# tangle-network/zk-SaaS

Measured on AMD Instinct MI355X. Metric: Groth16 proofs/sec (SHA-256 circuit), higher is better.
Workload: dtype u32 limbs (256-bit Montgomery); 1 GPU; BASELINE configs[3]: full distributed Groth16 on the SHA-256 circuit, BN254, l=2, n=8 parties on one GPU, all 12 masks sampled and applied (sha256.rs:226-291); masks=True, constraints=30006, wires=29823, domain=32768, len_a=14911, len_w=14911, len_u=16384, parties=8, packing_factor=2, fixed_base_tables=True

## Files before the change

### zk-saas_amd/csrc/msm.hpp

```cpp
#pragma once
#include <algorithm>
#include <atomic>
#include <cstdio>
#include <cstdlib>
#include <future>
#include <map>
#include <memory>
#include <mutex>
#include <type_traits>
#include <vector>

#include "ec.hpp"
#include "engine.hpp"
#include "msm_plan.hpp"
#include "ntt.hpp"
#include "quad.hpp"

namespace zk {
#if defined(__HIPCC__)

enum MsmRole { ROLE_SH, ROLE_W, ROLE_V, ROLE_U, NROLES };
constexpr const char* ROLE_NAME[NROLES] = {"S+H", "W", "V", "U"};
constexpr int NJOBS = 2;
constexpr int NBATCH = 3;
// ... 970 lines not shown
        k++;
        end_k = end_n;
        while (end_k == p + 1) {
          k++;
          end_k = offsets[k + 1];
        }
        end_n = offsets[k + 2 <= nkeys ? k + 2 : nkeys];
      }
    }
    e = e_next;
    pt = pt_next;
  }
}

constexpr int QUAD_THREADS = 256;
constexpr int QUAD_VL = QUAD_THREADS / 4;
inline int quad_threads(bool batched) {
  return batched ? 64 : 256;
}

template <class Fld>
__global__ __launch_bounds__(64) void msm_heavy_kernel(const XYZZ<Fld>* __restrict__ edge0, uint32_t nlanes, uint32_t tmin,
                                                       uint32_t cap, const uint32_t* __restrict__ offsets, uint32_t nkeys,
                                                       XYZZ<Fld>* __restrict__ buckets0,
                                                       const uint32_t* __restrict__ heavy,
                                                       XYZZ<Fld>* __restrict__ hpart0, uint32_t vcap, size_t ys) {
  __builtin_amdgcn_s_setprio(3);
  ZK_YSHIFT(offsets);
  ZK_YSHIFT(heavy);
  const uint32_t nh = heavy[1], V = heavy[0];
  if (blockIdx.x >= V) return;
  const XYZZ<Fld>* __restrict__ head = edge0 + (size_t)blockIdx.y * 2 * nlanes;
  const XYZZ<Fld>* __restrict__ tail = head + nlanes;
  XYZZ<Fld>* __restrict__ buckets = buckets0 + (size_t)blockIdx.y * nkeys;
  XYZZ<Fld>* __restrict__ hpart = hpart0 + (size_t)blockIdx.y * vcap;
  extern __shared__ uint4 smem_fin[];
  XYZZ<Fld>* sh = reinterpret_cast<XYZZ<Fld>*>(smem_fin);
  const uint32_t T = msm_range_len(offsets[nkeys], nlanes, tmin, cap);
  const int q = threadIdx.x & 3, vl = threadIdx.x >> 2;
  const int nq = (int)blockDim.x / 4;
  for (uint32_t v = blockIdx.x; v < V; v += gridDim.x) {
    uint32_t lo = 0, hi = nh;
    while (hi - lo > 1) {
      const uint32_t mid = (lo + hi) >> 1;
      if (heavy[3 + 2 * mid] <= v) lo = mid;
      else hi = mid;
    }
    const uint32_t kh = heavy[2 + 2 * lo], vb = heavy[3 + 2 * lo];
    const uint32_t S = (lo + 1 < nh ? heavy[3 + 2 * (lo + 1)] : V) - vb, s = v - vb;
    const uint32_t o0 = offsets[kh], o1 = offsets[kh + 1];
    const uint32_t l0 = o0 / T, l1 = (o1 - 1) / T;
    const uint32_t chunk = (l1 - l0 + S - 1) / S;
    const uint32_t first = l0 + 1 + s * chunk, last = first + chunk - 1 < l1 ? first + chunk - 1 : l1;
    Fld acc = (s == 0 && vl == 0) ? qload(tail + l0, q) : qidentity<Fld>(q);
    for (uint32_t l = first + (uint32_t)vl; l <= last; l += (uint32_t)nq) acc = qadd(acc, qload(head + l, q), q);
    acc = wg_quad_sum(acc, sh, vl, q, nq);
    if (vl == 0) qstore(S == 1 ? buckets + kh : hpart + v, q, acc);
    __syncthreads();
  }
}

constexpr int FIN_THREADS = 64;
template <class Fld>
__global__ __launch_bounds__(FIN_THREADS) void msm_finalize_kernel(const XYZZ<Fld>* __restrict__ edge0, uint32_t nlanes,
                                                               uint32_t tmin, uint32_t cap,
                                                               const uint32_t* __restrict__ offsets, uint32_t nkeys,
                                                               XYZZ<Fld>* __restrict__ buckets0,
                                                               const uint32_t* __restrict__ heavy,
                                                               const XYZZ<Fld>* __restrict__ hpart0, uint32_t vcap,
                                                               uint32_t fin_wgs, size_t ys) {
  __builtin_amdgcn_s_setprio(3);
  ZK_YSHIFT(offsets);
  const XYZZ<Fld>* __restrict__ head = edge0 + (size_t)blockIdx.y * 2 * nlanes;
  const XYZZ<Fld>* __restrict__ tail = head + nlanes;
  XYZZ<Fld>* __restrict__ buckets = buckets0 + (size_t)blockIdx.y * nkeys;
  const int q = threadIdx.x & 3;
  if (blockIdx.x >= fin_wgs) {
    ZK_YSHIFT(heavy);
    const uint32_t nh = heavy[1], V = heavy[0];
    const XYZZ<Fld>* __restrict__ hpart = hpart0 + (size_t)blockIdx.y * vcap;
    extern __shared__ uint4 smem_fin[];
    XYZZ<Fld>* sh = reinterpret_cast<XYZZ<Fld>*>(smem_fin);
    const int vl = threadIdx.x >> 2;
    for (uint32_t h = blockIdx.x - fin_wgs; h < nh; h += gridDim.x - fin_wgs) {
      const uint32_t vb = heavy[3 + 2 * h], S = (h + 1 < nh ? heavy[3 + 2 * (h + 1)] : V) - vb;
      if (S == 1) continue;
      Fld acc = qidentity<Fld>(q);
      for (uint32_t j = (uint32_t)vl; j < S; j += FIN_THREADS / 4) acc = qadd(acc, qload(hpart + vb + j, q), q);
      acc = wg_quad_sum(acc, sh, vl, q, FIN_THREADS / 4);
      if (vl == 0) qstore(buckets + heavy[2 + 2 * h], q, acc);
      __syncthreads();
    }
    return;
  }
  const uint32_t T = msm_range_len(offsets[nkeys], nlanes, tmin, cap);
  for (size_t k = (size_t)blockIdx.x * (FIN_THREADS / 4) + (threadIdx.x >> 2); k < nkeys;
       k += (size_t)fin_wgs * (FIN_THREADS / 4)) {
    const uint32_t o0 = offsets[k], o1 = offsets[k + 1];
    if (o0 == o1) {
      qstore(buckets + k, q, qidentity<Fld>(q));
      continue;
    }
    const uint32_t l0 = o0 / T, l1 = (o1 - 1) / T;
    if (l1 == l0 || l1 - l0 > FIN_SEQ) continue;
    Fld acc = qload(tail + l0, q);
    for (uint32_t l = l0 + 1; l <= l1; l++) acc = qadd(acc, qload(head + l, q), q);
    qstore(buckets + k, q, acc);
  }
}

template <class Fld>
__global__ __launch_bounds__(QUAD_THREADS, 2) void msm_reduce_a_kernel(const XYZZ<Fld>* __restrict__ buckets0, uint32_t B,
                                                                   int lo_bits, int nvl, XYZZ<Fld>* __restrict__ out0) {
  __builtin_amdgcn_s_setprio(3);
  extern __shared__ uint4 smem_red[];
  XYZZ<Fld>* sh = reinterpret_cast<XYZZ<Fld>*>(smem_red);
  const uint32_t LO = 1u << lo_bits, HI = B >> lo_bits;
  const uint32_t ngroups = HI + 1 + LO;
  const XYZZ<Fld>* __restrict__ wb = buckets0 + (size_t)blockIdx.y * B;
  const int q = threadIdx.x & 3, vl = threadIdx.x >> 2;
  const uint32_t g = blockIdx.x * (uint32_t)((int)blockDim.x / 4 / nvl) + (uint32_t)(vl / nvl);
  const uint32_t sub = (uint32_t)(vl & (nvl - 1));
  Fld acc = qidentity<Fld>(q);
  if (g <= HI) {
    for (uint32_t lo = sub; lo < LO; lo += (uint32_t)nvl) {
      uint32_t k = g * LO + lo;
      if (k >= 1 && k <= B) acc = qadd(acc, qload(wb + (k - 1), q), q);
    }
  } else if (g < ngroups) {
    const uint32_t lo = g - HI - 1;
    for (uint32_t hi = sub; hi <= HI; hi += (uint32_t)nvl) {
      uint32_t k = hi * LO + lo;
      if (k >= 1 && k <= B) acc = qadd(acc, qload(wb + (k - 1), q), q);
    }
  }
  acc = wg_quad_sum(acc, sh, vl, q, nvl);
  if (sub == 0 && g < ngroups) qstore(out0 + (size_t)blockIdx.y * ngroups + g, q, acc);
}

template <class Fld>
__global__ __launch_bounds__(QUAD_THREADS, 2) void msm_reduce_b_kernel(const XYZZ<Fld>* __restrict__ rc0, uint32_t B, int lo_bits,
                                                                   int nvl, XYZZ<Fld>* __restrict__ out0,
                                                                   const uint32_t* __restrict__ cnt_src, size_t cnt_stride,
                                                                   uint32_t ncnt, uint32_t* __restrict__ cnt_dst) {
  __builtin_amdgcn_s_setprio(3);
  if (blockIdx.x == 0 && blockIdx.y == 0 && threadIdx.x < ncnt)
    cnt_dst[2 * threadIdx.x] = *(const uint32_t*)((const char*)cnt_src + threadIdx.x * cnt_stride);
  extern __shared__ uint4 smem_red[];
  XYZZ<Fld>* sh = reinterpret_cast<XYZZ<Fld>*>(smem_red);
  const uint32_t LO = 1u << lo_bits, HI = B >> lo_bits;
  const uint32_t ngroups = HI + 1 + LO;
  int hb = 0;
  while ((1u << hb) < HI) hb++;
  const int nslices = hb + 1 + lo_bits;
  const XYZZ<Fld>* __restrict__ rc = rc0 + (size_t)blockIdx.y * ngroups;
  const int q = threadIdx.x & 3, vl = threadIdx.x >> 2;
  const int j = (int)blockIdx.x * ((int)blockDim.x / 4 / nvl) + vl / nvl;
  const uint32_t sub = (uint32_t)(vl & (nvl - 1));
  Fld acc = qidentity<Fld>(q);
  if (j <= hb) {
    for (uint32_t hi = sub; hi <= HI; hi += (uint32_t)nvl)
      if ((hi >> j) & 1u) acc = qadd(acc, qload(rc + hi, q), q);
  } else if (j < nslices) {
    const int jj = j - hb - 1;
    for (uint32_t lo = sub; lo < LO; lo += (uint32_t)nvl)
      if ((lo >> jj) & 1u) acc = qadd(acc, qload(rc + HI + 1 + lo, q), q);
  }
  acc = wg_quad_sum(acc, sh, vl, q, nvl);
  if (sub == 0 && j < nslices) qstore(out0 + (size_t)blockIdx.y * nslices + j, q, acc);
}

template <class Fld>
__global__ __launch_bounds__(128) void msm_table_kernel(const Affine<Fld>* __restrict__ bases, size_t len, int c,
                                                       int nwin, int wide, Affine<Fld>* __restrict__ table) {
  size_t i = (size_t)blockIdx.x * blockDim.x + threadIdx.x;
  if (i >= len) return;
  Affine<Fld> p = load_elem(bases + i);
  if (p.is_identity()) {
    for (int w = 0; w < nwin; w++) store_elem(table + (size_t)w * len + i, p);
    return;
  }
  XYZZ<Fld> acc = XYZZ<Fld>::from_affine(p);
  int left = 0;
  for (int w = 0; w < nwin;) {
    if (left == 0) {
      store_elem(table + (size_t)w * len + i, xyzz_to_affine(acc));
      left = w < wide ? c : c - 1;
      w++;
      if (w == nwin) break;
    }
    acc = xyzz_dbl(acc);
    left--;
  }
}

#endif

template <class Fld>
struct KernelField {
  using type = Fld;
};
template <class P>
struct KernelField<Fp2T<P, false>> {
  using type = Fp2T<P, (P::N <= ZK_MUL_INLINE_LIMBS)>;
};

struct MsmSlot {
  DevBuf ws;
  void* pinned = nullptr;
  size_t pinned_bytes = 0;
  hipEvent_t ev = nullptr;
  std::atomic<bool> busy{false};
  std::shared_ptr<const MsmTable> tab, tab2;
  hipError_t wait(const IEngine* eng) {
    if (!busy) return hipSuccess;
    hipError_t he = eng->event_wait(ev);
    if (he == hipErrorNotReady) return he;
    tab.reset();
    tab2.reset();
    busy = false;
    return he;
  }
// ... 426 lines not shown
```

### zk-saas_amd/csrc/msm_impl.hpp

```cpp
#pragma once
#include "msm.hpp"
#include "pack_split.hpp"

namespace zk {

#define MSM_HIP(x)                                           \
  do {                                                       \
    hipError_t _e = (x);                                     \
    if (_e != hipSuccess) return eng->hip_fail(_e, #x);      \
  } while (0)
#ifdef ZK_MSM_DEBUG_SYNC
#define MSM_STAGE(name)                                                          \
  do {                                                                           \
    hipError_t _e = hipStreamSynchronize(st);                                    \
    fprintf(stderr, "[zk msm] %s done (%s) npts=%zu c=%d nwin=%d\n", name,       \
            hipGetErrorString(_e), pl.npts, pl.win.c, pl.win.nwin);              \
    if (_e != hipSuccess) return eng->hip_fail(_e, name);                        \
  } while (0)
#else
#define MSM_STAGE(name) do { } while (0)
#endif

template <class Fr, class KF>
struct MsmViews {
// ... 104 lines not shown
                                           std::to_string(gate.sorted_cnt->load()) + " of " + std::to_string(gate.sorted_need) + ")");
    for (int i = 0; i < gate.n_wait_sorted; i++) MSM_HIP(hipStreamWaitEvent(st, gate.wait_sorted[i], 0));
  }
  if (gate.wait_ev) {
    if (gate.wait_flag && !eng->spin_until([&] { return gate.wait_flag->load(std::memory_order_acquire) != 0; }))
      return eng->fail(ZK_ERR_GENERIC, "msm launch: the accumulate kernel ahead of this one in the batch's chain was not enqueued within the deadline");
    MSM_HIP(hipStreamWaitEvent(st, gate.wait_ev, 0));
  }
  if constexpr (G2FLD) {
    msm_accumulate_split_kernel<typename BaseParams<Fld>::type><<<dim3((nlanes + 31) / 32, NB), dim3(128), 0, st>>>(
        bases, bases2, v.sorted, v.offsets, nkeys, nlanes, pl.tmin, pl.cap, v.buckets, v.edge, v.heavy, v.k0, pl.ys);
  } else {
    msm_accumulate_kernel<KF><<<dim3((nlanes + 127) / 128, NB), dim3(128), 0, st>>>(
        (const Affine<KF>*)bases, (const Affine<KF>*)bases2, v.sorted, v.offsets, nkeys, nlanes, pl.tmin, pl.cap, v.buckets,
        v.edge, v.heavy, v.k0, pl.ys, 0);
  }
  if (gate.signal_ev) {
    MSM_HIP(hipEventRecord(gate.signal_ev, st));
    if (gate.signal_flag) gate.signal_flag->store(1, std::memory_order_release);
  }
  return ZK_OK;
}

template <class Fr, class Fld, class KF>
int msm_stage_reduce(IEngine* eng, const MsmPlan& pl, const MsmViews<Fr, KF>& v, hipStream_t st) {
  constexpr bool G2FLD = IsExtField<Fld>::value;
  const unsigned NB = pl.vectors, nsets = (unsigned)pl.nsets;
  const uint32_t nkeys = (uint32_t)pl.nkeys, nlanes = pl.nlanes, tmin = pl.tmin, cap = pl.cap;
  const size_t ys = pl.ys;
  ProfScope ps_(eng->prof, G2FLD ? PROF_MSM_REDUCE_G2 : PROF_MSM_REDUCE, st, (double)pl.nkeys * NB);
  const int qt = quad_threads(pl.batch > 1), qvl = qt / 4;
  const size_t quad_lds = (size_t)qvl * sizeof(XYZZ<Fld>);
  msm_heavy_kernel<KF><<<dim3(2048, NB), dim3(64), (size_t)16 * sizeof(XYZZ<Fld>), st>>>(v.edge, nlanes, tmin, cap, v.offsets, nkeys,
                                                                    v.buckets, v.heavy, v.hpart, pl.vcap, ys);
  MSM_STAGE("heavy buckets");
  {
    const size_t fin_wgs = std::min<size_t>((pl.nkeys + FIN_THREADS / 4 - 1) / (FIN_THREADS / 4), 8192);
    const unsigned fin_extra = 256;
    msm_finalize_kernel<KF><<<dim3((unsigned)fin_wgs + fin_extra, NB), dim3(FIN_THREADS),
                              (size_t)(FIN_THREADS / 4) * sizeof(XYZZ<Fld>), st>>>(
        v.edge, nlanes, tmin, cap, v.offsets, nkeys, v.buckets, v.heavy, v.hpart, pl.vcap, (uint32_t)fin_wgs, ys);
  }
  MSM_STAGE("finalize");
  const size_t tot_groups = (size_t)pl.red_groups * NB * nsets;
  const size_t tot_slices = (size_t)pl.nslices * NB * nsets;
  const size_t cap_quads = (size_t)1024 * (G2FLD ? 2 : 3) * 16;
  auto pick_nvl = [&](size_t groups) {
    int n = qvl;
    while (n > 4 && groups * (size_t)n > cap_quads) n >>= 1;
    return n;
  };
  const int nvl_a = pick_nvl(tot_groups), nvl_b = pick_nvl(tot_slices);
  const unsigned gpw_a = (unsigned)(qvl / nvl_a), gpw_b = (unsigned)(qvl / nvl_b);
  msm_reduce_a_kernel<KF><<<dim3((pl.red_groups + gpw_a - 1) / gpw_a, NB * nsets), dim3((unsigned)qt), quad_lds, st>>>(
      v.buckets, pl.B, pl.lo_bits, nvl_a, v.rc);
  msm_reduce_b_kernel<KF><<<dim3(((unsigned)pl.nslices + gpw_b - 1) / gpw_b, NB * nsets), dim3((unsigned)qt), quad_lds, st>>>(
      v.rc, pl.B, pl.lo_bits, nvl_b, v.out,
      v.offsets + nkeys, ys, pl.nsorts, v.stats);
  return ZK_OK;
}

template <class FrP, class Fld>
int msm_launch(IEngine* eng, MsmSlot& slot, const MsmTuning& tune, const void* bases, const void* bases2,
               const void* scalars, size_t npts, const Fp<FrP>* coef_d, size_t part_len, hipStream_t st,
               MsmPending* pend, const MsmBatchArg* ba) {
  using Fr = Fp<FrP>;
  using KF = typename KernelField<Fld>::type;
  static_assert(sizeof(KF) == sizeof(Fld), "kernel field layout");
  static_assert(sizeof(XYZZ<Fld>) == 4 * sizeof(Fld), "the plan sizes XYZZ points as four coordinates");
  constexpr bool G2FLD = IsExtField<Fld>::value;
  *pend = MsmPending{};
  const unsigned NB = bases2 ? 2u : 1u;
  const void* const bases_in = bases;
  const void* const bases2_in = bases2;
  size_t toff = 0, toff2 = 0;
  std::shared_ptr<const MsmTable> tab = TableRegistry::inst().find(bases, npts, sizeof(Affine<Fld>), FrP::BITS, &toff), tab2;
  if (tab && NB == 2) {
    tab2 = TableRegistry::inst().find(bases2, npts, sizeof(Affine<Fld>), FrP::BITS, &toff2);
    if (!tab2 || tab2->len != tab->len || toff2 != toff || tab2->c != tab->c) tab = nullptr;
    else bases2 = tab2->data;
  }
  if (tab) bases = tab->data;
  MsmPlanIn in;
  in.scalar_bits = FrP::BITS, in.scalar_bytes = (int)sizeof(Fr), in.coord_bytes = (int)sizeof(Fld), in.g2 = G2FLD;
  if constexpr (G2FLD) in.acc_waves = SPLIT_WAVES<typename BaseParams<Fld>::type>;
  else in.acc_waves = ACC_WAVES<Fld>;
  in.npts = npts, in.batch = ba ? (size_t)ba->nb : 1, in.vectors = (int)NB;
  if (tab) {
    in.tab_c = tab->c, in.tab_len = tab->len, in.tab_off = toff;
    in.tab_no_identity = !tab->any_identity && (NB == 1 || !tab2->any_identity);
  }
  in.c_force = tune.c_force, in.bigsort_min = tune.bigsort_min;
  const MsmPlan pl = msm_plan(in);
  if (pl.err) return eng->fail(ZK_ERR_BAD_INPUT, pl.err);
  pend->fold = pl.fold;
  if (npts == 0) return ZK_OK;
  hipError_t he = slot.ws.ensure(pl.ws_bytes);
  if (he != hipSuccess) return eng->hip_fail(he, "msm workspace");
  he = slot.ensure_pinned(pl.pinned_bytes);
  if (he != hipSuccess) return eng->hip_fail(he, "msm pinned buffer");
  if (!slot.ev) {
    he = hipEventCreateWithFlags(&slot.ev, hipEventDisableTiming);
    if (he != hipSuccess) return eng->hip_fail(he, "msm event");
  }
  slot.busy = true;
  slot.tab = tab;
  slot.tab2 = tab2;
  pend->slot = &slot;
  struct RecordOnExit {
    MsmSlot& s;
// ... 92 lines not shown
```

### zk-saas_amd/csrc/quad.hpp

```cpp
#pragma once
#include "ec.hpp"
#include "ntt.hpp"

namespace zk {
#if defined(__HIPCC__)

template <int P0, int P1, int P2, int P3>
ZK_D uint32_t qperm_u32(uint32_t v) {
  return (uint32_t)__builtin_amdgcn_mov_dpp((int)v, P0 | (P1 << 2) | (P2 << 4) | (P3 << 6), 0xf, 0xf, true);
}
template <int P0, int P1, int P2, int P3, class P>
ZK_D Fp<P> qperm(const Fp<P>& v) {
  Fp<P> r;
#pragma unroll
  for (int i = 0; i < P::N; i++) r.v[i] = qperm_u32<P0, P1, P2, P3>(v.v[i]);
  return r;
}
template <int P0, int P1, int P2, int P3, class P, bool I>
ZK_D Fp2T<P, I> qperm(const Fp2T<P, I>& v) {
  return {qperm<P0, P1, P2, P3>(v.c0), qperm<P0, P1, P2, P3>(v.c1)};
}
template <class P>
ZK_D Fp<P> qsel(bool a, const Fp<P>& x, const Fp<P>& y) {
  Fp<P> r;
#pragma unroll
  for (int i = 0; i < P::N; i++) r.v[i] = a ? x.v[i] : y.v[i];
  return r;
}
template <class P, bool I>
ZK_D Fp2T<P, I> qsel(bool a, const Fp2T<P, I>& x, const Fp2T<P, I>& y) {
  return {qsel(a, x.c0, y.c0), qsel(a, x.c1, y.c1)};
}

template <class Fld>
ZK_D Fld qidentity(int q) {
  return q < 2 ? Fld::one() : Fld::zero();
}
template <class Fld>
ZK_D Fld qload(const XYZZ<Fld>* p, int q) {
  return load_elem(reinterpret_cast<const Fld*>(p) + q);
}
template <class Fld>
ZK_D void qstore(XYZZ<Fld>* p, int q, const Fld& c) {
  store_elem(reinterpret_cast<Fld*>(p) + q, c);
}

template <class Fld>
ZK_D Fld qadd(const Fld& ca, const Fld& cb, int q) {
  const bool even = (q & 1) == 0;
  const bool za = qperm<2, 2, 2, 2>(ca).is_zero();
  const bool zb = qperm<2, 2, 2, 2>(cb).is_zero();
  Fld A = qsel(even, qperm<0, 0, 1, 1>(ca), qperm<0, 0, 1, 1>(cb));
  Fld B = qsel(even, qperm<2, 2, 3, 3>(cb), qperm<2, 2, 3, 3>(ca));
  const Fld m1 = A * B;
  const Fld d = qperm<1, 1, 3, 3>(m1) - qperm<0, 0, 2, 2>(m1);
  const bool pz = qperm<0, 0, 0, 0>(d).is_zero();
  const bool rz = qperm<2, 2, 2, 2>(d).is_zero();
  const bool D = pz && rz && !za && !zb;
  const Fld cu = qsel(q == 1, ca.dbl(), ca);
  A = qsel(D, cu, qsel(even, d, qperm<0, 2, 2, 3>(ca)));
  B = qsel(D, cu, qsel(even, d, qperm<0, 2, 2, 3>(cb)));
  const Fld m2 = A * B;
  const Fld XX = qperm<0, 0, 0, 0>(m2);
  const Fld M = XX.dbl() + XX;
  A = qsel(D, qsel(q == 3, M, cu), qsel(q == 2, qperm<0, 1, 1, 3>(m2), qsel(q == 1, d, m1)));
  B = qsel(D, qsel(q == 3, M, qperm<1, 1, 1, 1>(m2)), XX);
  const Fld m3 = A * B;
  const Fld m3_1 = qperm<1, 1, 1, 1>(m3);
  const Fld m3_0 = qperm<0, 0, 0, 0>(m3);
  const Fld T = qsel(D, qperm<3, 3, 3, 3>(m3), qperm<2, 2, 2, 2>(m2)) - m3_0.dbl();
  const Fld X3f = qsel(D, T, T - m3_1);
  A = qsel(D, qsel(q == 0, M, m3_1),
           qsel(q == 1, qperm<2, 2, 2, 2>(d), qsel(q == 0, qperm<2, 2, 2, 2>(m1), m2)));
  B = qsel(D, qsel(q == 0, m3_0 - X3f, ca),
           qsel(q == 1, m3_0 - X3f, m3_1));
  const Fld m4 = A * B;
  const Fld m4_0 = qperm<0, 0, 0, 0>(m4), m4_1 = qperm<1, 1, 1, 1>(m4);
  const Fld Y3 = qsel(D, m4_0 - m4_1, m4_1 - m4_0);
  Fld r = qsel(q == 0, X3f, qsel(q == 1, Y3, qsel(q == 2, m3, m4)));
  if (pz && !rz) r = qidentity<Fld>(q);
  if (zb) r = ca;
  if (za) r = cb;
  return r;
}

template <class F>
ZK_D F cswap(const F& v) {
  return qperm<1, 0, 3, 2>(v);
}
template <class F>
ZK_D F hswap(const F& v) {
  return qperm<2, 3, 0, 1>(v);
}
template <class P>
ZK_D Fp<P> s2_mul(const Fp<P>& a, const Fp<P>& b, bool comp) {
  const Fp<P> ao = cswap(a), bo = cswap(b);
  return Fp<P>::mul_pm_mul(a, qsel(comp, bo, b), ao, qsel(comp, b, bo), comp);
}
template <class P>
ZK_D Fp<P> s2_sqr(const Fp<P>& a, bool comp) {
  const Fp<P> ao = cswap(a);
  return (a + qsel(comp, a, ao)) * qsel(comp, ao, a - ao);
}
template <class P>
ZK_D bool s2_is_zero(const Fp<P>& a) {
  const uint32_t z = a.is_zero() ? 1u : 0u;
  return (z & qperm_u32<1, 0, 3, 2>(z)) != 0;
}
template <class P>
struct SplitAcc {
  Fp<P> c0, c1;
};
template <class P>
ZK_D SplitAcc<P> split_identity(bool comp) {
  return SplitAcc<P>{qsel(comp, Fp<P>::zero(), Fp<P>::one()), Fp<P>::zero()};
}
template <class P>
ZK_D SplitAcc<P> split_madd(const SplitAcc<P>& a, const Fp<P>& in, bool half, bool comp) {
  using F = Fp<P>;
  const uint32_t zz = s2_is_zero(a.c1) ? 1u : 0u;
  SplitAcc<P> r;
  if (qperm_u32<0, 0, 0, 0>(zz)) {
    r.c0 = in;
    r.c1 = qsel(comp, F::zero(), F::one());
    return r;
  }
  const F m1 = s2_mul(in, a.c1, comp);
  const F d = m1 - a.c0;
  const F od = hswap(d);
  const uint32_t dz = s2_is_zero(d) ? 1u : 0u;
  const bool pz = qperm_u32<0, 0, 0, 0>(dz) != 0, rz = qperm_u32<2, 2, 2, 2>(dz) != 0;
  if (pz) {
    if (!rz) return split_identity<P>(comp);
    const F u = qsel(half, in.dbl(), in);
    const F m2 = s2_sqr(u, comp);
    const F o2 = hswap(m2);
// ... 46 lines not shown
  const Fp<P> ninv = (sq + cswap(sq)).inverse_fast();
  const Fp<P> r = z * ninv;
  return qsel(comp, r.neg(), r);
}
ZK_D bool quad_all(bool b) {
  uint32_t z = b ? 1u : 0u;
  z &= qperm_u32<1, 0, 3, 2>(z);
  z &= qperm_u32<2, 3, 0, 1>(z);
  return z != 0;
}
template <class P>
__device__ __noinline__ Fp<P> split_affine_add(const Fp<P>& a, bool ida, const Fp<P>& b, bool idb, bool half, bool comp,
                                               bool* idr) {
  using F = Fp<P>;
  *idr = false;
  if (ida) {
    *idr = idb;
    return b;
  }
  if (idb) return a;
  const F d = b - a;
  const uint32_t dz = s2_is_zero(d) ? 1u : 0u;
  const bool xz = qperm_u32<0, 0, 0, 0>(dz) != 0, yz = qperm_u32<2, 2, 2, 2>(dz) != 0;
  const F xa = qperm<0, 1, 0, 1>(a), ya = qperm<2, 3, 2, 3>(a);
  F lam;
  if (xz) {
    if (!yz) {
      *idr = true;
      return F::zero();
    }
    const F xx = s2_sqr(xa, comp);
    lam = s2_mul(xx.dbl() + xx, split_inv(ya.dbl(), comp), comp);
  } else {
    lam = s2_mul(qperm<2, 3, 2, 3>(d), split_inv(qperm<0, 1, 0, 1>(d), comp), comp);
  }
  const F x3 = s2_sqr(lam, comp) - xa - qperm<0, 1, 0, 1>(b);
  const F y3 = s2_mul(lam, xa - x3, comp) - ya;
  return qsel(half, y3, x3);
}

template <class P>
ZK_D void split_store_affine(const SplitAcc<P>& acc, Fp<P>* dst, bool half, bool comp) {
  using F = Fp<P>;
  const uint32_t zz = s2_is_zero(acc.c1) ? 1u : 0u;
  if (qperm_u32<0, 0, 0, 0>(zz)) {
    store_elem(dst, F::zero());
    return;
  }
  const F zi = split_inv(qperm<2, 3, 2, 3>(acc.c1), comp);
  const F zi2 = s2_sqr(s2_mul(zi, qperm<0, 1, 0, 1>(acc.c1), comp), comp);
  store_elem(dst, s2_mul(acc.c0, qsel(half, zi, zi2), comp));
}

template <class Fld>
ZK_D Fld wg_quad_sum(Fld c, XYZZ<Fld>* sh, int vl, int q, int nvl) {
  qstore(sh + vl, q, c);
  __syncthreads();
  for (int off = nvl >> 1; off >= 1; off >>= 1) {
    const bool act = (vl & (nvl - 1)) < off;
    Fld r = c;
    if (act) r = qadd(c, qload(sh + vl + off, q), q);
    __syncthreads();
    if (act) {
      c = r;
      qstore(sh + vl, q, c);
    }
    __syncthreads();
  }
  return c;
}

#endif
}
```

### zk-saas_amd/csrc/msm_plan.hpp

```cpp
#pragma once
#include <algorithm>
#include <cstddef>
#include <cstdint>

namespace zk {

constexpr size_t MSM_RANGE_MIN = 20, MSM_RANGE = 64;
constexpr size_t MSM_RANGE_MIN_G2 = 16, MSM_RANGE_G2 = 64;
constexpr uint32_t FIN_SEQ = 16;
constexpr int MSM_MAXB = 16;

constexpr int BIG_HI = 8;
constexpr int BIG_MAX_BINS = 8192;
constexpr int BIG_THREADS = 256;
constexpr int BIG_PTS_PER_THREAD = 8;
constexpr int BIG_EPT = 16;
constexpr size_t BIG_LDS_MAX = 156 * 1024;
inline int msm_big_hi(size_t nsets) {
  int hi = BIG_HI;
  while (hi > 0 && (nsets << hi) > (size_t)BIG_MAX_BINS) hi--;
  return hi;
}
constexpr size_t msm_bins_words(size_t nbins) { return 3 * nbins + 2; }

constexpr int ISCAN_THREADS = 256;
constexpr int ISCAN_PER = 8;
constexpr int ISCAN_BLOCK = ISCAN_THREADS * ISCAN_PER;

inline size_t msm_heavy_cap(size_t nlanes) { return nlanes / FIN_SEQ + 8; }
inline size_t msm_heavy_vcap(size_t nlanes) { return nlanes / FIN_SEQ + nlanes / 256 + 8; }

struct MsmWindows {
  int c = 0, nwin = 0, wide = 0;
  static MsmWindows of(int scalar_bits, int c_req) {
    const int T = scalar_bits + 1;
    MsmWindows w;
    w.nwin = (T + c_req - 1) / c_req;
    w.c = (T + w.nwin - 1) / w.nwin;
    w.wide = T - w.nwin * (w.c - 1);
    return w;
  }
  int width(int w) const { return w < wide ? c : c - 1; }
  int start(int w) const { return w * (c - 1) + std::min(w, wide); }
};

inline int msm_pick_c(int scalar_bits, size_t npts, int c_force = 0) {
  if (c_force >= 2 && c_force <= 20) return c_force;
  int best = 4;
  double best_cost = 1e300;
  for (int c = 4; c <= 20; c++) {
    int nwin = (scalar_bits + c) / c;
    int ceff = (scalar_bits + nwin) / nwin;
    double cost = (double)nwin * ((double)npts + (ceff > 17 ? 10.0 : 4.0) * (double)((size_t)1 << (ceff - 1)));
    if (cost <= best_cost) {
      best_cost = cost;
      best = c;
    }
  }
  return best;
}

struct MsmLanes {
  uint32_t nlanes, tmin, cap;
};
inline MsmLanes msm_pick_lanes(size_t max_entries, int waves, bool pair, int lanes_per_range = 0) {
  if (!lanes_per_range) lanes_per_range = pair ? 2 : 1;
  const size_t cap = (size_t)1024 * waves * (64 / lanes_per_range);
  const size_t lo = pair ? MSM_RANGE_MIN_G2 : MSM_RANGE_MIN;
  const size_t hi = pair ? MSM_RANGE_G2 : MSM_RANGE;
  size_t t = std::min(hi, std::max(lo, (size_t)((double)max_entries / (2.4 * (double)cap))));
  size_t nl = std::max<size_t>(1, (max_entries + t - 1) / t);
  if (max_entries >= cap * t && max_entries < 2 * cap * t && (max_entries + 2 * cap - 1) / (2 * cap) >= 12)
    nl = std::max(nl, 2 * cap);
  return MsmLanes{(uint32_t)nl, (uint32_t)t, (uint32_t)cap};
}

inline int table_c_auto(size_t len, bool g2) {
  if (g2) return len < ((size_t)1 << 20) ? 15 : 19;
  return len <= ((size_t)1 << 17) ? 15 : len < ((size_t)1 << 19) ? 16 : len < ((size_t)1 << 22) ? 18 : 20;
}
// ... 222 lines not shown
```

Before: 647.9 proofs/s.

## Unify MSM chain and tree reductions into a single qadd call site

Replaces the separate accumulate-loop plus wg_quad_sum tree reduction with quad_chain_tree_sum, a single loop in which each step performs one qadd, first over chained addends and then over the LDS tree. The two bucket-reduce kernels are merged into one stage-parameterized msm_reduce_kernel, and the finalize kernel's heavy and normal paths now share that loop. The likely aim is to inline the large qadd body once per kernel to cut code size and register pressure. A per-type FIN_WAVES occupancy hint is added to the finalize kernel's launch bounds. In exchange there is more predicated, divergent work per step and extra barriers in the finalize path.

```diff
diff --git a/zk-saas_amd/csrc/msm.hpp b/zk-saas_amd/csrc/msm.hpp
--- a/zk-saas_amd/csrc/msm.hpp
+++ b/zk-saas_amd/csrc/msm.hpp
@@ -1047,8 +1047,12 @@
     const uint32_t chunk = (l1 - l0 + S - 1) / S;
     const uint32_t first = l0 + 1 + s * chunk, last = first + chunk - 1 < l1 ? first + chunk - 1 : l1;
     Fld acc = (s == 0 && vl == 0) ? qload(tail + l0, q) : qidentity<Fld>(q);
-    for (uint32_t l = first + (uint32_t)vl; l <= last; l += (uint32_t)nq) acc = qadd(acc, qload(head + l, q), q);
-    acc = wg_quad_sum(acc, sh, vl, q, nq);
+    const uint32_t nchain = last >= first ? (last - first + (uint32_t)nq) / (uint32_t)nq : 0;
+    acc = quad_chain_tree_sum(acc, nchain, nq, sh, vl, q, [&](uint32_t i, bool* valid) {
+      const uint32_t l = first + (uint32_t)vl + i * (uint32_t)nq;
+      *valid = l <= last;
+      return head + l;
+    });
     if (vl == 0) qstore(S == 1 ? buckets + kh : hpart + v, q, acc);
     __syncthreads();
   }
@@ -1056,7 +1060,9 @@
 
 constexpr int FIN_THREADS = 64;
 template <class Fld>
-__global__ __launch_bounds__(FIN_THREADS) void msm_finalize_kernel(const XYZZ<Fld>* __restrict__ edge0, uint32_t nlanes,
+constexpr int FIN_WAVES = sizeof(Fld) <= 32 ? 4 : sizeof(Fld) <= 64 ? 2 : 1;
+template <class Fld>
+__global__ __launch_bounds__(FIN_THREADS, FIN_WAVES<Fld>) void msm_finalize_kernel(const XYZZ<Fld>* __restrict__ edge0, uint32_t nlanes,
                                                                uint32_t tmin, uint32_t cap,
                                                                const uint32_t* __restrict__ offsets, uint32_t nkeys,
                                                                XYZZ<Fld>* __restrict__ buckets0,
@@ -1065,80 +1071,58 @@
                                                                uint32_t fin_wgs, size_t ys) {
   __builtin_amdgcn_s_setprio(3);
   ZK_YSHIFT(offsets);
+  ZK_YSHIFT(heavy);
   const XYZZ<Fld>* __restrict__ head = edge0 + (size_t)blockIdx.y * 2 * nlanes;
   const XYZZ<Fld>* __restrict__ tail = head + nlanes;
   XYZZ<Fld>* __restrict__ buckets = buckets0 + (size_t)blockIdx.y * nkeys;
-  const int q = threadIdx.x & 3;
-  if (blockIdx.x >= fin_wgs) {
-    ZK_YSHIFT(heavy);
-    const uint32_t nh = heavy[1], V = heavy[0];
-    const XYZZ<Fld>* __restrict__ hpart = hpart0 + (size_t)blockIdx.y * vcap;
-    extern __shared__ uint4 smem_fin[];
-    XYZZ<Fld>* sh = reinterpret_cast<XYZZ<Fld>*>(smem_fin);
-    const int vl = threadIdx.x >> 2;
-    for (uint32_t h = blockIdx.x - fin_wgs; h < nh; h += gridDim.x - fin_wgs) {
-      const uint32_t vb = heavy[3 + 2 * h], S = (h + 1 < nh ? heavy[3 + 2 * (h + 1)] : V) - vb;
+  const XYZZ<Fld>* __restrict__ hpart = hpart0 + (size_t)blockIdx.y * vcap;
+  extern __shared__ uint4 smem_fin[];
+  XYZZ<Fld>* sh = reinterpret_cast<XYZZ<Fld>*>(smem_fin);
+  const int q = threadIdx.x & 3, vl = threadIdx.x >> 2;
+  constexpr uint32_t NQ = FIN_THREADS / 4;
+  const bool extra = blockIdx.x >= fin_wgs;
+  const uint32_t nh = extra ? heavy[1] : 0, V = extra ? heavy[0] : 0;
+  const uint32_t T = extra ? 1 : msm_range_len(offsets[nkeys], nlanes, tmin, cap);
+  const XYZZ<Fld>* __restrict__ from = extra ? hpart : head;
+  const uint32_t step = extra ? NQ : 1;
+  const uint32_t nitems = extra ? nh : nkeys, stride = extra ? gridDim.x - fin_wgs : fin_wgs * NQ;
+  for (uint32_t base = extra ? blockIdx.x - fin_wgs : blockIdx.x * NQ; base < nitems;
+       base = nitems - base > stride ? base + stride : nitems) {
+    uint32_t first = 0, nchain = 0, end = ~0u;
+    bool store = true;
+    Fld acc = qidentity<Fld>(q);
+    if (extra) {
+      const uint32_t vb = heavy[3 + 2 * base], S = (base + 1 < nh ? heavy[3 + 2 * (base + 1)] : V) - vb;
       if (S == 1) continue;
-      Fld acc = qidentity<Fld>(q);
-      for (uint32_t j = (uint32_t)vl; j < S; j += FIN_THREADS / 4) acc = qadd(acc, qload(hpart + vb + j, q), q);
-      acc = wg_quad_sum(acc, sh, vl, q, FIN_THREADS / 4);
-      if (vl == 0) qstore(buckets + heavy[2 + 2 * h], q, acc);
-      __syncthreads();
-    }
-    return;
-  }
-  const uint32_t T = msm_range_len(offsets[nkeys], nlanes, tmin, cap);
-  for (size_t k = (size_t)blockIdx.x * (FIN_THREADS / 4) + (threadIdx.x >> 2); k < nkeys;
-       k += (size_t)fin_wgs * (FIN_THREADS / 4)) {
-    const uint32_t o0 = offsets[k], o1 = offsets[k + 1];
-    if (o0 == o1) {
-      qstore(buckets + k, q, qidentity<Fld>(q));
-      continue;
-    }
-    const uint32_t l0 = o0 / T, l1 = (o1 - 1) / T;
-    if (l1 == l0 || l1 - l0 > FIN_SEQ) continue;
-    Fld acc = qload(tail + l0, q);
-    for (uint32_t l = l0 + 1; l <= l1; l++) acc = qadd(acc, qload(head + l, q), q);
-    qstore(buckets + k, q, acc);
+      first = vb + (uint32_t)vl, end = vb + S, nchain = (S + NQ - 1) / NQ;
+      store = vl == 0;
+    } else {
+      const uint32_t k = base + (uint32_t)vl;
+      const uint32_t o0 = k < nkeys ? offsets[k] : 0, o1 = k < nkeys ? offsets[k + 1] : 1;
+      if (k >= nkeys) store = false;
+      else if (o0 != o1) {
+        const uint32_t l0 = o0 / T, l1 = (o1 - 1) / T;
+        if (l1 == l0 || l1 - l0 > FIN_SEQ) store = false;
+        else acc = qload(tail + l0, q), first = l0 + 1, nchain = l1 - l0;
+      }
+    }
+    acc = quad_chain_tree_sum(acc, nchain, extra ? (int)NQ : 1, sh, vl, q, [&](uint32_t i, bool* valid) {
+      const uint32_t e = first + i * step;
+      *valid = e < end;
+      return from + e;
+    });
+    if (store) qstore(buckets + (extra ? heavy[2 + 2 * base] : base + (live_u32(threadIdx.x) >> 2)), q, acc);
+    if (extra) __syncthreads();
   }
 }
 
 template <class Fld>
-__global__ __launch_bounds__(QUAD_THREADS, 2) void msm_reduce_a_kernel(const XYZZ<Fld>* __restrict__ buckets0, uint32_t B,
-                                                                   int lo_bits, int nvl, XYZZ<Fld>* __restrict__ out0) {
+__global__ __launch_bounds__(QUAD_THREADS, 2) void msm_reduce_kernel(int stage, const XYZZ<Fld>* __restrict__ src0, uint32_t B,
+                                                                 int lo_bits, int nvl, XYZZ<Fld>* __restrict__ out0,
+                                                                 const uint32_t* __restrict__ cnt_src, size_t cnt_stride,
+                                                                 uint32_t ncnt, uint32_t* __restrict__ cnt_dst) {
   __builtin_amdgcn_s_setprio(3);
-  extern __shared__ uint4 smem_red[];
-  XYZZ<Fld>* sh = reinterpret_cast<XYZZ<Fld>*>(smem_red);
-  const uint32_t LO = 1u << lo_bits, HI = B >> lo_bits;
-  const uint32_t ngroups = HI + 1 + LO;
-  const XYZZ<Fld>* __restrict__ wb = buckets0 + (size_t)blockIdx.y * B;
-  const int q = threadIdx.x & 3, vl = threadIdx.x >> 2;
-  const uint32_t g = blockIdx.x * (uint32_t)((int)blockDim.x / 4 / nvl) + (uint32_t)(vl / nvl);
-  const uint32_t sub = (uint32_t)(vl & (nvl - 1));
-  Fld acc = qidentity<Fld>(q);
-  if (g <= HI) {
-    for (uint32_t lo = sub; lo < LO; lo += (uint32_t)nvl) {
-      uint32_t k = g * LO + lo;
-      if (k >= 1 && k <= B) acc = qadd(acc, qload(wb + (k - 1), q), q);
-    }
-  } else if (g < ngroups) {
-    const uint32_t lo = g - HI - 1;
-    for (uint32_t hi = sub; hi <= HI; hi += (uint32_t)nvl) {
-      uint32_t k = hi * LO + lo;
-      if (k >= 1 && k <= B) acc = qadd(acc, qload(wb + (k - 1), q), q);
-    }
-  }
-  acc = wg_quad_sum(acc, sh, vl, q, nvl);
-  if (sub == 0 && g < ngroups) qstore(out0 + (size_t)blockIdx.y * ngroups + g, q, acc);
-}
-
-template <class Fld>
-__global__ __launch_bounds__(QUAD_THREADS, 2) void msm_reduce_b_kernel(const XYZZ<Fld>* __restrict__ rc0, uint32_t B, int lo_bits,
-                                                                   int nvl, XYZZ<Fld>* __restrict__ out0,
-                                                                   const uint32_t* __restrict__ cnt_src, size_t cnt_stride,
-                                                                   uint32_t ncnt, uint32_t* __restrict__ cnt_dst) {
-  __builtin_amdgcn_s_setprio(3);
-  if (blockIdx.x == 0 && blockIdx.y == 0 && threadIdx.x < ncnt)
+  if (stage == 1 && blockIdx.x == 0 && blockIdx.y == 0 && threadIdx.x < ncnt)
     cnt_dst[2 * threadIdx.x] = *(const uint32_t*)((const char*)cnt_src + threadIdx.x * cnt_stride);
   extern __shared__ uint4 smem_red[];
   XYZZ<Fld>* sh = reinterpret_cast<XYZZ<Fld>*>(smem_red);
@@ -1146,22 +1130,38 @@
   const uint32_t ngroups = HI + 1 + LO;
   int hb = 0;
   while ((1u << hb) < HI) hb++;
-  const int nslices = hb + 1 + lo_bits;
-  const XYZZ<Fld>* __restrict__ rc = rc0 + (size_t)blockIdx.y * ngroups;
+  const uint32_t nslices = (uint32_t)(hb + 1 + lo_bits);
+  const uint32_t nout = stage == 0 ? ngroups : nslices;
+  const XYZZ<Fld>* __restrict__ src = src0 + (size_t)blockIdx.y * (stage == 0 ? B : ngroups);
   const int q = threadIdx.x & 3, vl = threadIdx.x >> 2;
-  const int j = (int)blockIdx.x * ((int)blockDim.x / 4 / nvl) + vl / nvl;
+  const int lg_nvl = 31 - __builtin_clz((unsigned)nvl);
+  const uint32_t longest = LO > HI + 1 ? LO : HI + 1;
+  auto group_of = [&](uint32_t tid) { return blockIdx.x * (blockDim.x >> (2 + lg_nvl)) + (tid >> (2 + lg_nvl)); };
   const uint32_t sub = (uint32_t)(vl & (nvl - 1));
-  Fld acc = qidentity<Fld>(q);
-  if (j <= hb) {
-    for (uint32_t hi = sub; hi <= HI; hi += (uint32_t)nvl)
-      if ((hi >> j) & 1u) acc = qadd(acc, qload(rc + hi, q), q);
-  } else if (j < nslices) {
-    const int jj = j - hb - 1;
-    for (uint32_t lo = sub; lo < LO; lo += (uint32_t)nvl)
-      if ((lo >> jj) & 1u) acc = qadd(acc, qload(rc + HI + 1 + lo, q), q);
-  }
-  acc = wg_quad_sum(acc, sh, vl, q, nvl);
-  if (sub == 0 && j < nslices) qstore(out0 + (size_t)blockIdx.y * nslices + j, q, acc);
+  uint32_t desc, fixed;
+  {
+    const uint32_t g = group_of(threadIdx.x);
+    const bool over_lo = stage == 0 ? g <= HI : g > (uint32_t)hb;
+    fixed = stage == 0 ? (over_lo ? g * LO : g - HI - 1) : (over_lo ? HI + 1 : 0);
+    const uint32_t bit = stage == 0 ? 0 : (over_lo ? g - (uint32_t)hb - 1 : g) & 31u;
+    desc = (g < nout ? 1u : 0u) | (over_lo ? 2u : 0u) | bit << 2;
+  }
+  Fld acc = quad_chain_tree_sum(qidentity<Fld>(q), (longest + (uint32_t)nvl - 1) >> lg_nvl, nvl, sh, vl, q,
+                                [&](uint32_t i, bool* valid) {
+    const uint32_t d = live_u32(desc);
+    const uint32_t e = sub + i * (uint32_t)nvl;
+    const bool over_lo = (d & 2u) != 0;
+    const bool in_group = (d & 1u) != 0 && e < (over_lo ? LO : HI + 1);
+    if (stage == 0) {
+      const uint32_t k = over_lo ? fixed + e : e * LO + fixed;
+      *valid = in_group && k >= 1 && k <= B;
+      return src + (k ? k - 1 : 0);
+    }
+    *valid = in_group && ((e >> (d >> 2)) & 1u);
+    return src + fixed + e;
+  });
+  const uint32_t g = group_of(live_u32(threadIdx.x));
+  if (sub == 0 && g < nout) qstore(out0 + (size_t)blockIdx.y * nout + g, q, acc);
 }
 
 template <class Fld>
diff --git a/zk-saas_amd/csrc/msm_impl.hpp b/zk-saas_amd/csrc/msm_impl.hpp
--- a/zk-saas_amd/csrc/msm_impl.hpp
+++ b/zk-saas_amd/csrc/msm_impl.hpp
@@ -180,10 +180,10 @@
   };
   const int nvl_a = pick_nvl(tot_groups), nvl_b = pick_nvl(tot_slices);
   const unsigned gpw_a = (unsigned)(qvl / nvl_a), gpw_b = (unsigned)(qvl / nvl_b);
-  msm_reduce_a_kernel<KF><<<dim3((pl.red_groups + gpw_a - 1) / gpw_a, NB * nsets), dim3((unsigned)qt), quad_lds, st>>>(
-      v.buckets, pl.B, pl.lo_bits, nvl_a, v.rc);
-  msm_reduce_b_kernel<KF><<<dim3(((unsigned)pl.nslices + gpw_b - 1) / gpw_b, NB * nsets), dim3((unsigned)qt), quad_lds, st>>>(
-      v.rc, pl.B, pl.lo_bits, nvl_b, v.out,
+  msm_reduce_kernel<KF><<<dim3((pl.red_groups + gpw_a - 1) / gpw_a, NB * nsets), dim3((unsigned)qt), quad_lds, st>>>(
+      0, v.buckets, pl.B, pl.lo_bits, nvl_a, v.rc, nullptr, 0, 0, nullptr);
+  msm_reduce_kernel<KF><<<dim3(((unsigned)pl.nslices + gpw_b - 1) / gpw_b, NB * nsets), dim3((unsigned)qt), quad_lds, st>>>(
+      1, v.rc, pl.B, pl.lo_bits, nvl_b, v.out,
       v.offsets + nkeys, ys, pl.nsorts, v.stats);
   return ZK_OK;
 }
diff --git a/zk-saas_amd/csrc/quad.hpp b/zk-saas_amd/csrc/quad.hpp
--- a/zk-saas_amd/csrc/quad.hpp
+++ b/zk-saas_amd/csrc/quad.hpp
@@ -234,22 +234,35 @@
   store_elem(dst, s2_mul(acc.c0, qsel(half, zi, zi2), comp));
 }
 
-template <class Fld>
-ZK_D Fld wg_quad_sum(Fld c, XYZZ<Fld>* sh, int vl, int q, int nvl) {
-  qstore(sh + vl, q, c);
-  __syncthreads();
-  for (int off = nvl >> 1; off >= 1; off >>= 1) {
-    const bool act = (vl & (nvl - 1)) < off;
-    Fld r = c;
-    if (act) r = qadd(c, qload(sh + vl + off, q), q);
-    __syncthreads();
+ZK_D uint32_t live_u32(uint32_t v) {
+  asm volatile("" : "+v"(v));
+  return v;
+}
+
+template <class Fld, class Addend>
+ZK_D Fld quad_chain_tree_sum(Fld acc, uint32_t nchain, int nvl, XYZZ<Fld>* sh, int vl, int q, Addend&& addend) {
+  const uint32_t sub = (uint32_t)(vl & (nvl - 1));
+  const uint32_t nsteps = nchain + (uint32_t)(31 - __builtin_clz((unsigned)nvl));
+  for (uint32_t step = 0; step < nsteps; step++) {
+    const bool tree = step >= nchain;
+    bool act;
+    Fld b;
+    if (tree) {
+      const uint32_t off = (uint32_t)nvl >> (step - nchain + 1);
+      act = sub < off;
+      if (step == nchain) qstore(sh + vl, q, acc);
+      __syncthreads();
+      b = act ? qload(sh + vl + off, q) : acc;
+    } else {
+      const XYZZ<Fld>* p = addend(step, &act);
+      b = act ? qload(p, q) : acc;
+    }
     if (act) {
-      c = r;
-      qstore(sh + vl, q, c);
+      acc = qadd(acc, b, q);
+      if (tree) qstore(sh + vl, q, acc);
     }
-    __syncthreads();
-  }
-  return c;
+  }
+  return acc;
 }
 
 #endif
```

Result: slower. 629.2 proofs/s (-2.9%).

## Streamline quad XYZZ add, skip identity adds, and enumerate bit-slice indices directly

Applied to the files above, without the earlier changes.

Rewrites qadd so the rare doubling case branches to a separate noinline qdbl instead of blending both paths through qsel in every multiply, and merges the zero checks into single lane permutes. Adds qaccum, which takes the first loaded element directly instead of adding it to an identity. The reduce_b kernel now iterates only over indices with bit j set, using closed-form slice index and count helpers, rather than scanning every index and testing the bit. This trades some divergence and call overhead on the doubling path for fewer field multiplies and fewer wasted loop iterations in the MSM bucket reductions.

```diff
diff --git a/zk-saas_amd/csrc/msm.hpp b/zk-saas_amd/csrc/msm.hpp
--- a/zk-saas_amd/csrc/msm.hpp
+++ b/zk-saas_amd/csrc/msm.hpp
@@ -1046,8 +1046,9 @@
     const uint32_t l0 = o0 / T, l1 = (o1 - 1) / T;
     const uint32_t chunk = (l1 - l0 + S - 1) / S;
     const uint32_t first = l0 + 1 + s * chunk, last = first + chunk - 1 < l1 ? first + chunk - 1 : l1;
-    Fld acc = (s == 0 && vl == 0) ? qload(tail + l0, q) : qidentity<Fld>(q);
-    for (uint32_t l = first + (uint32_t)vl; l <= last; l += (uint32_t)nq) acc = qadd(acc, qload(head + l, q), q);
+    bool have = s == 0 && vl == 0;
+    Fld acc = have ? qload(tail + l0, q) : qidentity<Fld>(q);
+    for (uint32_t l = first + (uint32_t)vl; l <= last; l += (uint32_t)nq) qaccum(acc, have, head + l, q);
     acc = wg_quad_sum(acc, sh, vl, q, nq);
     if (vl == 0) qstore(S == 1 ? buckets + kh : hpart + v, q, acc);
     __syncthreads();
@@ -1080,7 +1081,8 @@
       const uint32_t vb = heavy[3 + 2 * h], S = (h + 1 < nh ? heavy[3 + 2 * (h + 1)] : V) - vb;
       if (S == 1) continue;
       Fld acc = qidentity<Fld>(q);
-      for (uint32_t j = (uint32_t)vl; j < S; j += FIN_THREADS / 4) acc = qadd(acc, qload(hpart + vb + j, q), q);
+      bool have = false;
+      for (uint32_t j = (uint32_t)vl; j < S; j += FIN_THREADS / 4) qaccum(acc, have, hpart + vb + j, q);
       acc = wg_quad_sum(acc, sh, vl, q, FIN_THREADS / 4);
       if (vl == 0) qstore(buckets + heavy[2 + 2 * h], q, acc);
       __syncthreads();
@@ -1116,16 +1118,17 @@
   const uint32_t g = blockIdx.x * (uint32_t)((int)blockDim.x / 4 / nvl) + (uint32_t)(vl / nvl);
   const uint32_t sub = (uint32_t)(vl & (nvl - 1));
   Fld acc = qidentity<Fld>(q);
+  bool have = false;
   if (g <= HI) {
     for (uint32_t lo = sub; lo < LO; lo += (uint32_t)nvl) {
       uint32_t k = g * LO + lo;
-      if (k >= 1 && k <= B) acc = qadd(acc, qload(wb + (k - 1), q), q);
+      if (k >= 1 && k <= B) qaccum(acc, have, wb + (k - 1), q);
     }
   } else if (g < ngroups) {
     const uint32_t lo = g - HI - 1;
     for (uint32_t hi = sub; hi <= HI; hi += (uint32_t)nvl) {
       uint32_t k = hi * LO + lo;
-      if (k >= 1 && k <= B) acc = qadd(acc, qload(wb + (k - 1), q), q);
+      if (k >= 1 && k <= B) qaccum(acc, have, wb + (k - 1), q);
     }
   }
   acc = wg_quad_sum(acc, sh, vl, q, nvl);
@@ -1152,13 +1155,14 @@
   const int j = (int)blockIdx.x * ((int)blockDim.x / 4 / nvl) + vl / nvl;
   const uint32_t sub = (uint32_t)(vl & (nvl - 1));
   Fld acc = qidentity<Fld>(q);
+  bool have = false;
   if (j <= hb) {
-    for (uint32_t hi = sub; hi <= HI; hi += (uint32_t)nvl)
-      if ((hi >> j) & 1u) acc = qadd(acc, qload(rc + hi, q), q);
+    const uint32_t cnt = msm_slice_count(HI + 1, j);
+    for (uint32_t t = sub; t < cnt; t += (uint32_t)nvl) qaccum(acc, have, rc + msm_slice_index(t, j), q);
   } else if (j < nslices) {
     const int jj = j - hb - 1;
-    for (uint32_t lo = sub; lo < LO; lo += (uint32_t)nvl)
-      if ((lo >> jj) & 1u) acc = qadd(acc, qload(rc + HI + 1 + lo, q), q);
+    const uint32_t cnt = msm_slice_count(LO, jj);
+    for (uint32_t t = sub; t < cnt; t += (uint32_t)nvl) qaccum(acc, have, rc + HI + 1 + msm_slice_index(t, jj), q);
   }
   acc = wg_quad_sum(acc, sh, vl, q, nvl);
   if (sub == 0 && j < nslices) qstore(out0 + (size_t)blockIdx.y * nslices + j, q, acc);
diff --git a/zk-saas_amd/csrc/msm_plan.hpp b/zk-saas_amd/csrc/msm_plan.hpp
--- a/zk-saas_amd/csrc/msm_plan.hpp
+++ b/zk-saas_amd/csrc/msm_plan.hpp
@@ -26,6 +26,19 @@
 constexpr int ISCAN_THREADS = 256;
 constexpr int ISCAN_PER = 8;
 constexpr int ISCAN_BLOCK = ISCAN_THREADS * ISCAN_PER;
+
+#if defined(__HIPCC__)
+#define ZK_PLAN_HD __host__ __device__
+#else
+#define ZK_PLAN_HD
+#endif
+ZK_PLAN_HD constexpr uint32_t msm_slice_index(uint32_t t, int j) {
+  return ((t >> j) << (j + 1)) | (1u << j) | (t & ((1u << j) - 1u));
+}
+ZK_PLAN_HD constexpr uint32_t msm_slice_count(uint32_t n, int j) {
+  const uint32_t rem = n & ((2u << j) - 1u);
+  return ((n >> (j + 1)) << j) + (rem > (1u << j) ? rem - (1u << j) : 0u);
+}
 
 inline size_t msm_heavy_cap(size_t nlanes) { return nlanes / FIN_SEQ + 8; }
 inline size_t msm_heavy_vcap(size_t nlanes) { return nlanes / FIN_SEQ + nlanes / 256 + 8; }
diff --git a/zk-saas_amd/csrc/quad.hpp b/zk-saas_amd/csrc/quad.hpp
--- a/zk-saas_amd/csrc/quad.hpp
+++ b/zk-saas_amd/csrc/quad.hpp
@@ -46,42 +46,56 @@
 }
 
 template <class Fld>
+__device__ __noinline__ Fld qdbl(Fld ca, int q) {
+  const Fld cu = qsel(q == 1, ca.dbl(), ca);
+  const Fld m2 = cu * cu;
+  const Fld XX = qperm<0, 0, 0, 0>(m2);
+  const Fld M = XX.dbl() + XX;
+  const Fld m3 = qsel(q == 3, M, cu) * qsel(q == 3, M, qperm<1, 1, 1, 1>(m2));
+  const Fld W = qperm<1, 1, 1, 1>(m3), S = qperm<0, 0, 0, 0>(m3);
+  const Fld X3 = qperm<3, 3, 3, 3>(m3) - S.dbl();
+  const Fld m4 = qsel(q == 0, M, W) * qsel(q == 0, S - X3, ca);
+  const Fld Y3 = qperm<0, 0, 0, 0>(m4) - qperm<1, 1, 1, 1>(m4);
+  return qsel(q == 0, X3, qsel(q == 1, Y3, qsel(q == 2, m3, m4)));
+}
+
+template <class Fld>
 ZK_D Fld qadd(const Fld& ca, const Fld& cb, int q) {
   const bool even = (q & 1) == 0;
-  const bool za = qperm<2, 2, 2, 2>(ca).is_zero();
-  const bool zb = qperm<2, 2, 2, 2>(cb).is_zero();
+  const uint32_t zab = qperm_u32<2, 2, 2, 2>((ca.is_zero() ? 1u : 0u) | (cb.is_zero() ? 2u : 0u));
+  const bool za = (zab & 1u) != 0, zb = (zab & 2u) != 0;
   Fld A = qsel(even, qperm<0, 0, 1, 1>(ca), qperm<0, 0, 1, 1>(cb));
   Fld B = qsel(even, qperm<2, 2, 3, 3>(cb), qperm<2, 2, 3, 3>(ca));
   const Fld m1 = A * B;
   const Fld d = qperm<1, 1, 3, 3>(m1) - qperm<0, 0, 2, 2>(m1);
-  const bool pz = qperm<0, 0, 0, 0>(d).is_zero();
-  const bool rz = qperm<2, 2, 2, 2>(d).is_zero();
-  const bool D = pz && rz && !za && !zb;
-  const Fld cu = qsel(q == 1, ca.dbl(), ca);
-  A = qsel(D, cu, qsel(even, d, qperm<0, 2, 2, 3>(ca)));
-  B = qsel(D, cu, qsel(even, d, qperm<0, 2, 2, 3>(cb)));
+  const uint32_t dz = d.is_zero() ? 1u : 0u;
+  const bool pz = qperm_u32<0, 0, 0, 0>(dz) != 0, rz = qperm_u32<2, 2, 2, 2>(dz) != 0;
+  if (pz && rz && !za && !zb) return qdbl(ca, q);
+  A = qsel(even, d, qperm<0, 2, 2, 3>(ca));
+  B = qsel(even, d, qperm<0, 2, 2, 3>(cb));
   const Fld m2 = A * B;
-  const Fld XX = qperm<0, 0, 0, 0>(m2);
-  const Fld M = XX.dbl() + XX;
-  A = qsel(D, qsel(q == 3, M, cu), qsel(q == 2, qperm<0, 1, 1, 3>(m2), qsel(q == 1, d, m1)));
-  B = qsel(D, qsel(q == 3, M, qperm<1, 1, 1, 1>(m2)), XX);
-  const Fld m3 = A * B;
+  A = qsel(q == 2, qperm<0, 1, 1, 3>(m2), qsel(q == 1, d, m1));
+  const Fld m3 = A * qperm<0, 0, 0, 0>(m2);
   const Fld m3_1 = qperm<1, 1, 1, 1>(m3);
   const Fld m3_0 = qperm<0, 0, 0, 0>(m3);
-  const Fld T = qsel(D, qperm<3, 3, 3, 3>(m3), qperm<2, 2, 2, 2>(m2)) - m3_0.dbl();
-  const Fld X3f = qsel(D, T, T - m3_1);
-  A = qsel(D, qsel(q == 0, M, m3_1),
-           qsel(q == 1, qperm<2, 2, 2, 2>(d), qsel(q == 0, qperm<2, 2, 2, 2>(m1), m2)));
-  B = qsel(D, qsel(q == 0, m3_0 - X3f, ca),
-           qsel(q == 1, m3_0 - X3f, m3_1));
+  const Fld X3f = qperm<2, 2, 2, 2>(m2) - m3_0.dbl() - m3_1;
+  A = qsel(q == 1, qperm<2, 2, 2, 2>(d), qsel(q == 0, qperm<2, 2, 2, 2>(m1), m2));
+  B = qsel(q == 1, m3_0 - X3f, m3_1);
   const Fld m4 = A * B;
-  const Fld m4_0 = qperm<0, 0, 0, 0>(m4), m4_1 = qperm<1, 1, 1, 1>(m4);
-  const Fld Y3 = qsel(D, m4_0 - m4_1, m4_1 - m4_0);
+  const Fld Y3 = qperm<1, 1, 1, 1>(m4) - qperm<0, 0, 0, 0>(m4);
   Fld r = qsel(q == 0, X3f, qsel(q == 1, Y3, qsel(q == 2, m3, m4)));
   if (pz && !rz) r = qidentity<Fld>(q);
   if (zb) r = ca;
   if (za) r = cb;
   return r;
+}
+
+template <class Fld>
+ZK_D void qaccum(Fld& acc, bool& have, const XYZZ<Fld>* p, int q) {
+  const Fld e = qload(p, q);
+  if (have) acc = qadd(acc, e, q);
+  else acc = e;
+  have = true;
 }
 
 template <class F>
```

Result: faster. 643.0 proofs/s before, 682.3 proofs/s after (median of 6 runs) (+6.1%).
